# bananaofhappiness/soundscope

Hardware: AMD Instinct MI355X
Metric: audio samples/s analyzed (48 kHz stereo) (higher is better)
Workload: dtype f32 + f64

## Files before the change

soundscope_amd/csrc/ss_fft.hip:

```cpp
#include "ss_kernels.h"
#include "ss_fft_dev.h"
#include <cstdlib>
#include <type_traits>

namespace ssk {

constexpr int kFftPairwWaves = 3;
constexpr int kFftWaves = 2;

constexpr int kX2Stride = 17;
constexpr int kRowB = 17;
constexpr int kPlaneB = 16 * kRowB;
#define X1B(ka, tb_, ta_) ((ka) * kPlaneB + (tb_) * kRowB + (ta_))
#define X2B(kb, ka_, tb_) ((kb) * kPlaneB + (ka_) * kRowB + (tb_))

#define SPEC_POS(k) ((k) ^ (((k) >> 5) & 3))

constexpr uint32_t kColStride = 516;
typedef __attribute__((address_space(3))) float lds_f32;
typedef __attribute__((address_space(3))) char lds_char;
__device__ __forceinline__ void lds_fmax(lds_f32 *p, float v) { (void)__hip_atomic_fetch_max(p, v, __ATOMIC_RELAXED, __HIP_MEMORY_SCOPE_WORKGROUP); }
template <bool LDS_TABLE = false, bool COLS = false>
__device__ __forceinline__ void fft4096_epilogue(const v2f *xb, int t, uint32_t first_bin, uint32_t n_bins,
                                                 float db_offset, const float *__restrict__ offpink,
                                                 float *o_mid, float *o_side, bool store_side = true,
                                                 float side_off = 0.0f, float *colbuf = nullptr, const uint2 *coltab = nullptr,
                                                 const uint2 *colbins = nullptr)
{
    const uint32_t ngroups = (n_bins + 3) >> 2;
    constexpr float kDb = 3.01029995663981195f;
    const float lg0 = __uint_as_float((uint32_t)__builtin_amdgcn_readfirstlane((int)__float_as_uint((-150.0f - db_offset) / kDb)));
    float4 op[2];
#pragma unroll
    for (int i = 0; i < 2; i++) {
        const uint32_t g = (uint32_t)t + 256u * i;
        op[i] = make_float4(0.f, 0.f, 0.f, 0.f);
        uint32_t boff = 16u * g;
        asm volatile("" : "+v"(boff));
        if (!LDS_TABLE && g < ngroups) op[i] = *reinterpret_cast<const float4 *>(reinterpret_cast<const char *>(offpink) + boff);
    }
    float rm[2][4], rs[2][4];
    lds_char *const cb = (lds_char *)colbuf;
    auto fold_group = [&](const int i, const uint32_t g) {
                const uint2 ct = coltab[g];
                const uint32_t o0 = ct.x & 0xFFFFu, o3 = ct.x >> 16, nf = ct.y;
                const bool general = nf == 0u;
                if (__builtin_expect(__ballot(general) != 0ull, 0)) {
                    if (general) {
                        uint32_t gg = g;
                        asm volatile("" : "+v"(gg));
                        const uint2 cw = colbins[gg];
                        const uint32_t o[4] = {cw.x & 0xFFFFu, cw.x >> 16, cw.y & 0xFFFFu, cw.y >> 16};
#pragma unroll
                        for (int e = 0; e < 4; e++) {
                            lds_f32 *a = (lds_f32 *)(cb + o[e]);
                            lds_fmax(a, rm[i][e]);
                            lds_fmax(a + kColStride, rs[i][e]);
                        }
                    }
                }
                if (!general) {
                    const bool p1 = nf > 1u, p2 = nf > 2u, p3 = nf > 3u;
                    auto max3 = [](float a, float b, float c) -> float { float r; asm("v_max3_f32 %0, %1, %2, %3" : "=v"(r) : "v"(a), "v"(b), "v"(c)); return r; };
                    auto max2 = [](float a, float b) -> float { float r; asm("v_max_f32 %0, %1, %2" : "=v"(r) : "v"(a), "v"(b)); return r; };
#pragma unroll
                    for (int row = 0; row < 2; row++) {
                        const float *r = row ? rs[i] : rm[i];
                        float f = max3(r[0], p1 ? r[1] : r[0], p2 ? r[2] : r[0]);
                        f = max2(f, p3 ? r[3] : r[0]);
                        const float l = max3(r[3], p2 ? r[3] : r[2], p1 ? r[3] : r[1]);
                        lds_fmax((lds_f32 *)(cb + o0) + row * kColStride, f);
                        if (!p3) lds_fmax((lds_f32 *)(cb + o3) + row * kColStride, l);
                    }
                }
    };
#pragma unroll
    for (int i = 0; i < 2; i++) {
        const uint32_t g = (uint32_t)t + 256u * i;
        if (g < ngroups) {
            uint32_t k0 = first_bin + 4 * g;
            if (COLS && i == 1) asm volatile("" : "+v"(k0));
            v2f zk[4], zm[4];
#pragma unroll
            for (int e = 0; e < 4; e++) {
                const uint32_t k = k0 + e;
                zk[e] = xb[SPEC_POS(k)];
                zm[e] = xb[SPEC_POS(4096 - k)];
            }
            if (LDS_TABLE) op[i] = reinterpret_cast<const float4 *>(offpink)[g];
#if defined(__HIP_DEVICE_COMPILE__)
            __builtin_amdgcn_sched_barrier(0);
#endif
            float qm[4], qs[4];
#pragma unroll
            for (int e = 0; e < 4; e++) {
                v2f P = zk[e] + zm[e], Q, t, qq;
                asm("v_pk_add_f32 %0, %1, %2 op_sel:[1,1] op_sel_hi:[0,0] neg_lo:[0,1] neg_hi:[0,1]" : "=v"(Q) : "v"(zk[e]), "v"(zm[e]));
                asm("v_pk_mul_f32 %0, %1, %1" : "=v"(t) : "v"(Q));
                asm("v_pk_fma_f32 %0, %1, %1, %2" : "=v"(qq) : "v"(P), "v"(t));
                qm[e] = qq.x;
                qs[e] = qq.y;
            }
            const float opv[4] = {op[i].x, op[i].y, op[i].z, op[i].w};
            const v2f so2 = {side_off, side_off};
            const v2f osa = v2f{op[i].x, op[i].y} + so2, osb = v2f{op[i].z, op[i].w} + so2;
            const float ops[4] = {osa.x, osa.y, osb.x, osb.y};
            const float qmin = fminf(fminf(fminf(qm[0], qm[1]), fminf(qm[2], qm[3])), fminf(fminf(qs[0], qs[1]), fminf(qs[2], qs[3])));
            if (__builtin_expect(__ballot(qmin == 0.0f) == 0ull, 1)) {
#pragma unroll
                for (int e = 0; e < 4; e++) {
                    rm[i][e] = fmaf(__log2f(qm[e]), kDb, opv[e]);
                    rs[i][e] = fmaf(__log2f(qs[e]), kDb, ops[e]);
                }
            } else {
#pragma unroll
                for (int e = 0; e < 4; e++) {
                    rm[i][e] = fmaf(qm[e] == 0.0f ? lg0 : __log2f(qm[e]), kDb, opv[e]);
                    rs[i][e] = qs[e] == 0.0f ? fmaf(lg0, kDb, opv[e]) : fmaf(__log2f(qs[e]), kDb, ops[e]);
                }
            }
            if (COLS) fold_group(i, g);
        } else {
#pragma unroll
            for (int e = 0; e < 4; e++) { rm[i][e] = 0.0f; rs[i][e] = 0.0f; }
        }
    }
    if (COLS) return;
#if defined(__HIP_DEVICE_COMPILE__)
    __builtin_amdgcn_sched_barrier(0);
#endif
#pragma unroll
    for (int i = 0; i < 2; i++) {
        const uint32_t g = (uint32_t)t + 256u * i;
        if (g < ngroups) {
            reinterpret_cast<float4 *>(o_mid)[g] = make_float4(rm[i][0], rm[i][1], rm[i][2], rm[i][3]);
            if (store_side) reinterpret_cast<float4 *>(o_side)[g] = make_float4(rs[i][0], rs[i][1], rs[i][2], rs[i][3]);
        }
    }
}

__device__ __forceinline__ void fft4096_nan_rows(int t, uint32_t n_bins, float *o_first, float *o_second, bool first_nan, bool second_nan)
{
    const uint32_t ngroups = (n_bins + 3) >> 2;
    __builtin_amdgcn_s_waitcnt(0);
    const float qn = __builtin_nanf("");
    for (uint32_t g = (uint32_t)t; g < ngroups; g += 256u) {
        if (first_nan) reinterpret_cast<float4 *>(o_first)[g] = make_float4(qn, qn, qn, qn);
        if (second_nan) reinterpret_cast<float4 *>(o_second)[g] = make_float4(qn, qn, qn, qn);
    }
}

__device__ __forceinline__ void fft4096_floor_rows(int t, uint32_t n_bins, float db_offset, const float *__restrict__ offpink,
                                                float *o_first, float *o_second, bool first_zero, bool second_zero)
{
    const uint32_t ngroups = (n_bins + 3) >> 2;
    __builtin_amdgcn_s_waitcnt(0);
    for (uint32_t g = (uint32_t)t; g < ngroups; g += 256u) {
        const float4 op = *reinterpret_cast<const float4 *>(offpink + 4 * g);
        const float4 v = make_float4(-150.0f + (op.x - db_offset), -150.0f + (op.y - db_offset), -150.0f + (op.z - db_offset), -150.0f + (op.w - db_offset));
        if (first_zero) reinterpret_cast<float4 *>(o_first)[g] = v;
        if (second_zero) reinterpret_cast<float4 *>(o_second)[g] = v;
    }
}

__device__ __forceinline__ void fft4096_floor_columns(int t, uint32_t n_bins, float db_offset, const float *__restrict__ offpink,
                                                      float *colbuf, const uint16_t *bincol, const float *col_init, uint32_t cols,
                                                      bool first_zero, bool second_zero)
{
    __syncthreads();
    for (uint32_t c = (uint32_t)t; c < cols; c += 256u) {
        if (first_zero) colbuf[c] = col_init[c];
        if (second_zero) colbuf[kColStride + c] = col_init[c];
    }
    __syncthreads();
    for (uint32_t k = (uint32_t)t; k < n_bins; k += 256u) {
        const uint32_t c = bincol[k];
        const float v = -150.0f + (offpink[k] - db_offset);
        if (first_zero) lds_fmax((lds_f32 *)colbuf + c, v);
        if (second_zero) lds_fmax((lds_f32 *)colbuf + kColStride + c, v);
    }
}

__device__ __forceinline__ uint32_t umax(uint32_t a, uint32_t b) { return a > b ? a : b; }
__device__ __forceinline__ uint32_t wave_umax_lane63(uint32_t v)
{
#define SS_UMAX_DPP(ctrl, rows) v = umax(v, (uint32_t)__builtin_amdgcn_update_dpp(0, (int)v, ctrl, rows, 0xF, true))
    SS_UMAX_DPP(0x111, 0xF);
    SS_UMAX_DPP(0x112, 0xF);
    SS_UMAX_DPP(0x114, 0xF);
    SS_UMAX_DPP(0x118, 0xF);
    SS_UMAX_DPP(0x142, 0xA);
    SS_UMAX_DPP(0x143, 0xC);
#undef SS_UMAX_DPP
    return v;
}
__device__ __forceinline__ float wave_fsum_lane63(float v)
{
#define SS_FSUM_DPP(ctrl, rows) v += __int_as_float(__builtin_amdgcn_update_dpp(0, __float_as_int(v), ctrl, rows, 0xF, true))
    SS_FSUM_DPP(0x111, 0xF);
    SS_FSUM_DPP(0x112, 0xF);
    SS_FSUM_DPP(0x114, 0xF);
    SS_FSUM_DPP(0x118, 0xF);
    SS_FSUM_DPP(0x142, 0xA);
    SS_FSUM_DPP(0x143, 0xC);
#undef SS_FSUM_DPP
    return v;
}
__device__ __forceinline__ int block_exp_energy(uint32_t a, uint32_t b)
{
    const int e = ((int)a - (int)b + (1 << 23)) >> 24;
    return e < -60 ? -60 : (e > 60 ? 60 : e);
}
__device__ __forceinline__ void read_energies2(const uint32_t (*lv)[2], uint32_t &a, uint32_t &b)
{
    const uint4 q0 = *reinterpret_cast<const uint4 *>(&lv[0][0]), q1 = *reinterpret_cast<const uint4 *>(&lv[2][0]);
    const float sa = (__uint_as_float(q0.x) + __uint_as_float(q0.z)) + (__uint_as_float(q1.x) + __uint_as_float(q1.z));
    const float sb = (__uint_as_float(q0.y) + __uint_as_float(q0.w)) + (__uint_as_float(q1.y) + __uint_as_float(q1.w));
    a = (uint32_t)__builtin_amdgcn_readfirstlane((int)__float_as_uint(sa));
    b = (uint32_t)__builtin_amdgcn_readfirstlane((int)__float_as_uint(sb));
}
__device__ __forceinline__ int block_exp(uint32_t a, uint32_t b)
{
    const int e = ((int)a - (int)b + (1 << 22)) >> 23;
    return e < -60 ? -60 : (e > 60 ? 60 : e);
}
__device__ __forceinline__ float exp2i(int e) { return __uint_as_float((uint32_t)(127 + e) << 23); }
__device__ __forceinline__ float uniform_f(float v) { return __uint_as_float((uint32_t)__builtin_amdgcn_readfirstlane((int)__float_as_uint(v))); }
__device__ __forceinline__ float block_off(int e) { return uniform_f((float)e * -6.02059991327962390f); }
__device__ __forceinline__ void read_levels2(const uint32_t (*lv)[2], uint32_t &a, uint32_t &b)
{
    const uint4 q0 = *reinterpret_cast<const uint4 *>(&lv[0][0]), q1 = *reinterpret_cast<const uint4 *>(&lv[2][0]);
    a = (uint32_t)__builtin_amdgcn_readfirstlane((int)umax(umax(q0.x, q0.z), umax(q1.x, q1.z)));
    b = (uint32_t)__builtin_amdgcn_readfirstlane((int)umax(umax(q0.y, q0.w), umax(q1.y, q1.w)));
}
__device__ __forceinline__ void read_levels4(const uint32_t (*lv)[8], uint32_t (&x)[4])
{
    const uint4 q0 = *reinterpret_cast<const uint4 *>(&lv[0][0]), q1 = *reinterpret_cast<const uint4 *>(&lv[1][0]);
    const uint4 q2 = *reinterpret_cast<const uint4 *>(&lv[2][0]), q3 = *reinterpret_cast<const uint4 *>(&lv[3][0]);
    x[0] = (uint32_t)__builtin_amdgcn_readfirstlane((int)umax(umax(q0.x, q1.x), umax(q2.x, q3.x)));
    x[1] = (uint32_t)__builtin_amdgcn_readfirstlane((int)umax(umax(q0.y, q1.y), umax(q2.y, q3.y)));
    x[2] = (uint32_t)__builtin_amdgcn_readfirstlane((int)umax(umax(q0.z, q1.z), umax(q2.z, q3.z)));
    x[3] = (uint32_t)__builtin_amdgcn_readfirstlane((int)umax(umax(q0.w, q1.w), umax(q2.w, q3.w)));
}
__device__ __forceinline__ void read_energies4(const uint32_t (*lv)[8], uint32_t (&g)[4])
{
    const uint4 e0 = *reinterpret_cast<const uint4 *>(&lv[0][4]), e1 = *reinterpret_cast<const uint4 *>(&lv[1][4]);
    const uint4 e2 = *reinterpret_cast<const uint4 *>(&lv[2][4]), e3 = *reinterpret_cast<const uint4 *>(&lv[3][4]);
    auto fs = [](uint32_t a, uint32_t b, uint32_t c, uint32_t d) -> uint32_t {
        return (uint32_t)__builtin_amdgcn_readfirstlane((int)__float_as_uint((__uint_as_float(a) + __uint_as_float(b)) + (__uint_as_float(c) + __uint_as_float(d))));
    };
    g[0] = fs(e0.x, e1.x, e2.x, e3.x); g[1] = fs(e0.y, e1.y, e2.y, e3.y);
    g[2] = fs(e0.z, e1.z, e2.z, e3.z); g[3] = fs(e0.w, e1.w, e2.w, e3.w);
}
__device__ __forceinline__ int exact_block_exp(uint32_t xa, uint32_t xb, uint32_t ga, uint32_t gb)
{
    if (xa == 0u || xb == 0u) return 0;
    const bool gok = ga != 0u && gb != 0u && ga < 0x7F800000u && gb < 0x7F800000u;
    return gok ? block_exp_energy(ga, gb) : block_exp(xa, xb);
}

// ... 169 lines not shown
struct PhaseMark {
    uint64_t pt = __builtin_amdgcn_s_memtime(), acc[12] = {0, 0, 0, 0, 0, 0, 0, 0, 0, 0, 0, 0};
    __device__ __forceinline__ void operator()(int i) { const uint64_t n = __builtin_amdgcn_s_memtime(); acc[i] += n - pt; pt = n; }
    __device__ __forceinline__ void end() const
    {
        if ((threadIdx.x & 63) != 0) return;
#pragma unroll
        for (int i = 0; i < 12; i++) atomicAdd(&g_fft_prof[i], (unsigned long long)acc[i]);
        atomicAdd(&g_fft_prof[15], 1ull);
    }
};
#else
typedef NoMark PhaseMark;
#endif

template <bool PRIO>
__device__ __forceinline__ void r16_fft(v2f (&z)[16])
{
    if (PRIO) SS_PRIO_LO();
    fft16(z);
    if (PRIO) SS_PRIO_HI();
}
template <class Mark>
__device__ __forceinline__ void r16_row_load(v2f (&z)[16], const v2f *row, Mark &mark, int i)
{
#pragma unroll
    for (int j = 0; j < 16; j++) z[j] = lds_ld64(&row[j]);
    mark(i);
    __syncthreads();
    mark(i + 1);
}
template <bool PRIO, class Mark>
__device__ __forceinline__ void r16_pass2(v2f (&z)[16], const v2f *row, v2f *x2, const v2f *twp, Mark &mark)
{
    r16_row_load(z, row, mark, 2);
    r16_fft<PRIO>(z);
    x2[0] = z[R16(0)];
    v2f twa[4], twb[4];
#pragma unroll
    for (int j = 0; j < 4; j++) twa[j] = lds_ld64(&twp[16 * (1 + j)]);
#pragma unroll
    for (int g = 0; g < 4; g++) {
        const int kb0 = 1 + 4 * g, nk = g == 3 ? 3 : 4;
        if (g < 3) {
#pragma unroll
            for (int j = 0; j < 4; j++) if (kb0 + 4 + j < 16) twb[j] = lds_ld64(&twp[16 * (kb0 + 4 + j)]);
        }
        __builtin_amdgcn_sched_barrier(0);
#pragma unroll
        for (int j = 0; j < nk; j++) x2[(kb0 + j) * kPlaneB] = pk_cmul(z[R16(kb0 + j)], twa[j]);
        __builtin_amdgcn_sched_barrier(0);
#pragma unroll
        for (int j = 0; j < 4; j++) twa[j] = twb[j];
    }
}

constexpr int kMs1Tw = 12;
template <int HS, int TWN, bool COLS>
__global__ __launch_bounds__(256, 3) void k_fft4096_ms1(FftBatchParams p)
{
    constexpr int NH = 16 / HS;
    __shared__ __attribute__((aligned(16))) v2f xbuf[16 * kPlaneB];
    __shared__ __attribute__((aligned(16))) v2f tw2s[256];
    __shared__ __attribute__((aligned(16))) uint32_t hoplev[NH][4][2];
    __shared__ __attribute__((aligned(16))) uint32_t xlev[4][2];
    __shared__ __attribute__((aligned(16))) float offp[2048];
    __shared__ __attribute__((aligned(16))) uint2 coltab[COLS ? 512 : 1];
    __shared__ __attribute__((aligned(16))) float colbuf[COLS ? 2 * kColStride : 1];
    const int t = threadIdx.x;
    WindowRun run;
    if (!window_run(p, run)) return;
    const uint32_t stream = run.stream, w_begin = run.begin, w_end = run.end;
    const float2 *src = reinterpret_cast<const float2 *>(p.pcm) + (size_t)stream * p.frames_per_stream +
                        p.first_start + (size_t)w_begin * p.hop;
    const v2f *twn = reinterpret_cast<const v2f *>(p.tw_n);
    v2f hwp[8];
#pragma unroll
    for (int j = 0; j < 8; j++) hwp[j] = v2f{p.half_window[t + 256 * (2 * j)], p.half_window[t + 256 * (2 * j + 1)]};
    v2f tw1[16];
    r16_load_tw1<TWN>(tw1, twn, t);
    tw2s[t] = reinterpret_cast<const v2f *>(p.tw_256)[(t & 15) * (t >> 4)];
    if (COLS) {
        for (uint32_t g = (uint32_t)t; 4u * g < p.bin_stride; g += 256u) coltab[g] = p.col_groups[g];
        for (uint32_t c = (uint32_t)t; c < p.cols; c += 256u) { const float v = p.col_init[c]; colbuf[c] = v; colbuf[kColStride + c] = v; }
        if (t < 4) { colbuf[512 + t] = 0.0f; colbuf[kColStride + 512 + t] = 0.0f; }
    }
    for (uint32_t g = (uint32_t)t; 4u * g < p.bin_stride; g += 256u)
        reinterpret_cast<float4 *>(offp)[g] = reinterpret_cast<const float4 *>(p.offpink)[g];
    const float cgain = COLS ? (p.integrated ? -13.0f - (float)p.integrated[stream] : p.gain_db) : 0.0f;
    auto flush_columns = [&](uint32_t wdone) {
        float *oc = p.out_cols + ((size_t)stream * p.n_windows + wdone) * 2u * p.cols;
        for (uint32_t c = (uint32_t)t; c < 2u * p.cols; c += 256u) {
            const uint32_t i = c < p.cols ? c : c - p.cols + kColStride;
            const float k = colbuf[i];
            const bool none = k != k;
            if (!none) colbuf[i] = -INFINITY;
            oc[c] = none ? k : fminf(fmaxf(k + cgain, -100.0f), 0.0f);
        }
    };
    const int tb = t & 15, hi = t >> 4;
    const int tsw = SPEC_POS(t);
    const size_t out_win_stride = (size_t)2 * p.bin_stride;
    float *outp = p.out + ((size_t)stream * p.n_windows + w_begin) * out_win_stride;
    v2f sd[16];
#pragma unroll
    for (int j = 0; j < 16; j++) sd[j] = pk_sum_diff(reinterpret_cast<const v2f *>(src)[t + 256 * j]);
    auto windowed = [&](int j) -> v2f { return (j & 1) ? pk_mul_bcast<1>(sd[j], hwp[j >> 1]) : pk_mul_bcast<0>(sd[j], hwp[j >> 1]); };
    const uint32_t wvid = (uint32_t)__builtin_amdgcn_readfirstlane(t >> 6);
    const bool lane63 = (t & 63) == 63;
#pragma unroll
    for (int g = 0; g < NH; g++) {
        float m = 0.0f, d = 0.0f;
#pragma unroll
        for (int q = 0; q < HS; q++) { m = fmaxf(m, fabsf(sd[g * HS + q].x)); d = fmaxf(d, fabsf(sd[g * HS + q].y)); }
        const uint32_t wm = wave_umax_lane63(__float_as_uint(m)), wd = wave_umax_lane63(__float_as_uint(d));
        if (lane63) *reinterpret_cast<uint2 *>(hoplev[(g + 1) % NH][wvid]) = make_uint2(wm, wd);
    }
    __syncthreads();
    uint32_t Pm[NH], Pd[NH];
    Pm[0] = 0u; Pd[0] = 0u;
#pragma unroll
    for (int g = 1; g < NH; g++) read_levels2(hoplev[g], Pm[g], Pd[g]);
    int E = 0;
    float scE = 1.0f, soffE = 0.0f;
    auto rescale = [&](int T) -> float {
        const int dE = T - E;
        if (dE < 2 && dE > -2) return 1.0f;
        const float sc = exp2i(dE);
#pragma unroll
        for (int j = 0; j < 16; j++) sd[j].y *= sc;
        E = T; scE = exp2i(E); soffE = block_off(E);
        return sc;
    };
    bool inner_ok = false;
    uint32_t thr_m = 0u, thr_d = 0u;
    auto presettle = [&]() {
        uint32_t mm = 0u, md = 0u;
#pragma unroll
        for (int g = 2; g < NH; g++) { mm = umax(mm, Pm[g]); md = umax(md, Pd[g]); }
        thr_m = mm + 0x800000u; thr_d = md + 0x800000u;
        inner_ok = mm != 0u && md != 0u && Pm[1] <= thr_m && Pd[1] <= thr_d;
        if (mm != 0u && md != 0u) rescale(block_exp(mm, md));
    };
    presettle();
    PhaseMark mark;
    for (uint32_t w = w_begin; w < w_end; ++w) {
        float2 nx[HS];
        const bool more = (w + 1 < w_end);
        if (COLS && w != w_begin) flush_columns(w - 1);
        const uint4 lq0 = *reinterpret_cast<const uint4 *>(&hoplev[0][0][0]), lq1 = *reinterpret_cast<const uint4 *>(&hoplev[0][2][0]);
        __builtin_amdgcn_sched_barrier(0);
        v2f z[16];
#pragma unroll
        for (int j = 0; j < 16; j++) z[j] = windowed(j);
        __builtin_amdgcn_sched_barrier(0);
        const uint32_t nPm = (uint32_t)__builtin_amdgcn_readfirstlane((int)umax(umax(lq0.x, lq0.z), umax(lq1.x, lq1.z)));
        const uint32_t nPd = (uint32_t)__builtin_amdgcn_readfirstlane((int)umax(umax(lq0.y, lq0.w), umax(lq1.y, lq1.w)));
#pragma unroll
        for (int g = 0; g < NH - 1; g++) { Pm[g] = Pm[g + 1]; Pd[g] = Pd[g + 1]; }
        Pm[NH - 1] = nPm; Pd[NH - 1] = nPd;
        bool zrow_m = false, zrow_d = false;
        if (__builtin_expect(!inner_ok || nPm > thr_m || nPd > thr_d, 0)) {
            uint32_t am = 0u, ad = 0u;
#pragma unroll
            for (int g = 0; g < NH; g++) { am |= Pm[g]; ad |= Pd[g]; }
            zrow_m = am == 0u; zrow_d = ad == 0u;
            if (!(zrow_m || zrow_d)) {
                float xm = 0.0f, xd = 0.0f;
#pragma unroll
                for (int j = 0; j < 16; j++) { xm = fmaf(z[j].x, z[j].x, xm); xd = fmaf(z[j].y, z[j].y, xd); }
                const float wm = wave_fsum_lane63(xm), wd = wave_fsum_lane63(xd);
                if (lane63) *reinterpret_cast<uint2 *>(xlev[wvid]) = make_uint2(__float_as_uint(wm), __float_as_uint(wd));
                __syncthreads();
                uint32_t Xm, Xd;
                read_energies2(xlev, Xm, Xd);
                if (Xm != 0u && Xd != 0u && Xm < 0x7F800000u && Xd < 0x7F800000u) {
                    int T = E + block_exp_energy(Xm, Xd);
                    T = T < -60 ? -60 : (T > 60 ? 60 : T);
                    const float sc = rescale(T);
#pragma unroll
                    for (int j = 0; j < 16; j++) z[j].y *= sc;
                }
            }
        }
        const float soff = soffE;
        r16_fft<true>(z);
        xbuf[X1B(0, tb, hi)] = z[R16(0)];
#pragma unroll
        for (int ka = 1; ka < 16; ka++) xbuf[X1B(ka, tb, hi)] = r16_pass1_tw<TWN>(ka, z[R16(ka)], tw1);
#pragma unroll
        for (int q = 0; q < HS; q++) {
            nx[q] = make_float2(0.f, 0.f);
            if (more) nx[q] = src[(size_t)(w + 1 - w_begin) * p.hop + t + 256 * (16 - HS + q)];
        }
        mark(0);
        __syncthreads();
        mark(1);
        r16_pass2<true>(z, &xbuf[X1B(hi, tb, 0)], &xbuf[X2B(0, hi, tb)], tw2s + tb, mark);
        mark(4);
        __syncthreads();
        mark(5);
        r16_row_load(z, &xbuf[X1B(hi, tb, 0)], mark, 6);
        r16_fft<true>(z);
#pragma unroll
        for (int kc = 0; kc < 16; kc++)
            if ((p.publish_mask >> kc) & 1u) xbuf[kc * 256 + tsw] = z[R16(kc)];
        mark(8);
        __syncthreads();
        mark(9);
        SS_PRIO_LO();
        if (more) {
#pragma unroll
            for (int j = 0; j < 16 - HS; j++) sd[j] = sd[j + HS];
            float m = 0.0f, d = 0.0f;
#pragma unroll
            for (int q = 0; q < HS; q++) {
                const v2f v = pk_sum_diff(v2f{nx[q].x, nx[q].y});
                m = fmaxf(m, fabsf(v.x)); d = fmaxf(d, fabsf(v.y));
                sd[16 - HS + q] = v2f{v.x, v.y * scE};
            }
            const uint32_t wm = wave_umax_lane63(__float_as_uint(m)), wd = wave_umax_lane63(__float_as_uint(d));
            if (lane63) *reinterpret_cast<uint2 *>(hoplev[0][wvid]) = make_uint2(wm, wd);
            presettle();
        }
        float *o_mid = outp + (size_t)(w - w_begin) * out_win_stride;
        fft4096_epilogue<true, COLS>(xbuf, t, p.first_bin, p.n_bins, p.db_offset, offp, o_mid, o_mid + p.bin_stride, true, soff, colbuf, coltab, p.col_bins);
        if (__builtin_expect(zrow_m || zrow_d, 0) && xbuf[SPEC_POS(p.first_bin)].x == xbuf[SPEC_POS(p.first_bin)].x) {
            if (!COLS) fft4096_floor_rows(t, p.n_bins, p.db_offset, p.offpink, o_mid, o_mid + p.bin_stride, zrow_m, zrow_d);
            else fft4096_floor_columns(t, p.n_bins, p.db_offset, p.offpink, colbuf, p.bin_col, p.col_init, p.cols, zrow_m, zrow_d);
        }
        mark(10);
        __syncthreads();
        mark(11);
    }
    mark.end();
    if (COLS) flush_columns(w_end - 1);
}

__global__ __launch_bounds__(256, kFftPairwWaves) void k_fft4096_pairw(FftBatchParams p, uint32_t fft_ch)
{
    __shared__ __attribute__((aligned(16))) v2f xbuf[16 * kPlaneB];
    __shared__ __attribute__((aligned(16))) v2f tw2s[256];
    __shared__ __attribute__((aligned(16))) uint32_t hoplev[5][4];
    __shared__ __attribute__((aligned(16))) uint32_t xlev[4][2];
    const int t = threadIdx.x;
    const uint32_t pairs_per_block = p.windows_per_block >> 1;
    const uint32_t n_pairs_max = (p.n_windows + 1) >> 1;
    const uint32_t groups = (n_pairs_max + pairs_per_block - 1) / pairs_per_block;
    uint32_t bid = xcd_logical_id();
    if (bid >= p.n_streams * groups * fft_ch) return;
    const uint32_t ch = bid % fft_ch; bid /= fft_ch;
    const uint32_t grp = bid % groups;
    const uint32_t stream = bid / groups;
    const uint32_t n_win = p.windows_of ? p.windows_of[stream] : p.n_windows;
    const uint32_t n_pairs = (n_win + 1) >> 1;
    const uint32_t pp_begin = grp * pairs_per_block;
    uint32_t pp_end = pp_begin + pairs_per_block;
    if (pp_begin >= n_pairs) return;
    if (pp_end > n_pairs) pp_end = n_pairs;
    const uint32_t C = p.channels;
    const float *src = p.pcm + ((size_t)stream * p.frames_per_stream + p.first_start + (size_t)pp_begin * 2048u) * C + ch;
    const v2f *twn = reinterpret_cast<const v2f *>(p.tw_n);
    float hw[16], hw2[16];
#pragma unroll
    for (int j = 0; j < 16; j++) hw2[j] = hw[j] = p.window[t + 256 * j];
    v2f tw1[16];
    r16_load_tw1<6>(tw1, twn, t);
    tw1[5] = twn[5 * t]; tw1[6] = twn[6 * t]; tw1[7] = twn[7 * t];
    tw2s[t] = reinterpret_cast<const v2f *>(p.tw_256)[(t & 15) * (t >> 4)];
    const int tb = t & 15, hi = t >> 4;
    const int tsw = SPEC_POS(t);
    const size_t row_stride = (size_t)fft_ch * p.bin_stride;
    float *outp = p.out + (((size_t)stream * p.n_windows + 2u * pp_begin) * fft_ch + ch) * p.bin_stride;
    float raw[20];
    const bool two0 = (2u * pp_begin + 1u < n_win);
#pragma unroll
    for (int j = 0; j < 20; j++) raw[j] = (j < 16 || two0) ? src[(size_t)(t + 256 * j) * C] : 0.0f;
    const uint32_t wvid = (uint32_t)__builtin_amdgcn_readfirstlane(t >> 6);
    const bool lane63 = (t & 63) == 63;
    auto hop_level = [&](float a, float b, float c, float d) -> uint32_t {
        const uint32_t ua = __float_as_uint(a) & 0x7FFFFFFFu, ub = __float_as_uint(b) & 0x7FFFFFFFu;
        const uint32_t uc = __float_as_uint(c) & 0x7FFFFFFFu, ud = __float_as_uint(d) & 0x7FFFFFFFu;
        return wave_umax_lane63(umax(umax(ua, ub), umax(uc, ud)));
    };
    auto read_level = [&](const uint32_t *lv) -> uint32_t {
        const uint4 q = *reinterpret_cast<const uint4 *>(lv);
        return (uint32_t)__builtin_amdgcn_readfirstlane((int)umax(umax(q.x, q.y), umax(q.z, q.w)));
    };
#pragma unroll
    for (int g = 0; g < 5; g++) {
        const uint32_t wl = hop_level(raw[4 * g], raw[4 * g + 1], raw[4 * g + 2], raw[4 * g + 3]);
        if (lane63) hoplev[g][wvid] = wl;
    }
    __syncthreads();
    uint32_t P[5];
#pragma unroll
    for (int g = 0; g < 5; g++) P[g] = read_level(hoplev[g]);
    int E = 0;
    auto settle = [&]() {
        if ((P[0] | P[1] | P[2] | P[3]) == 0u || (P[1] | P[2] | P[3] | P[4]) == 0u) return;
        if (umax(umax(umax(P[0], P[1]), umax(P[2], P[3])), P[4]) >= 0x7F800000u) return;
        const uint32_t ma = umax(P[1], P[2]), ea = umax(P[0], P[3]), mb = umax(P[2], P[3]), eb = umax(P[1], P[4]);
        int T;
        if (ma != 0u && mb != 0u && ea <= ma + 0x800000u && eb <= mb + 0x800000u) {
            T = block_exp(ma, mb);
        } else {
            float xa = 0.0f, xb = 0.0f;
#pragma unroll
            for (int j = 0; j < 16; j++) { const float pa = raw[j] * hw[j], pb = raw[j + 4] * hw[j]; xa = fmaf(pa, pa, xa); xb = fmaf(pb, pb, xb); }
            const float wa = wave_fsum_lane63(xa), wb = wave_fsum_lane63(xb);
            if (lane63) *reinterpret_cast<uint2 *>(xlev[wvid]) = make_uint2(__float_as_uint(wa), __float_as_uint(wb));
            __syncthreads();
            uint32_t Xa, Xb;
            read_energies2(xlev, Xa, Xb);
            if (Xa == 0u || Xb == 0u || Xa >= 0x7F800000u || Xb >= 0x7F800000u) return;
            T = block_exp_energy(Xa, Xb);
        }
        const int dE = T - E;
        if (dE >= 2 || dE <= -2) {
            const float sc = exp2i(T);
#pragma unroll
            for (int j = 0; j < 16; j++) hw2[j] = hw[j] * sc;
            E = T;
        }
    };
    settle();
    NoMark nomark;
    for (uint32_t pp = pp_begin; pp < pp_end; ++pp) {
        const bool two = (2u * pp + 1u < n_win);
        const bool more = (pp + 1 < pp_end);
        const bool more2 = more && (2u * pp + 3u < n_win);
        const bool zrow_a = (P[0] | P[1] | P[2] | P[3]) == 0u, zrow_b = (P[1] | P[2] | P[3] | P[4]) == 0u;
        float nx[8];
        const float *nsrc = src + ((size_t)(pp - pp_begin) * 2048u + t) * C;
#pragma unroll
        for (int q = 0; q < 8; q++) {
            nx[q] = 0.0f;
            if (q < 4 ? more : more2) nx[q] = nsrc[(size_t)(256 * (20 + q)) * C];
        }
// ... 678 lines not shown
```

soundscope_amd/csrc/ss_fft_dev.h:

```cpp
#pragma once
#include "ss_kernels.h"

namespace ssk {

__device__ __forceinline__ float2 cadd(float2 a, float2 b) { return make_float2(a.x + b.x, a.y + b.y); }
__device__ __forceinline__ float2 csub(float2 a, float2 b) { return make_float2(a.x - b.x, a.y - b.y); }
__device__ __forceinline__ float2 cmul(float2 a, float2 w) { return make_float2(a.x * w.x - a.y * w.y, a.x * w.y + a.y * w.x); }
__device__ __forceinline__ float2 cmul_cs(float2 a, float c, float s) { return make_float2(a.x * c + a.y * s, a.y * c - a.x * s); }
__device__ __forceinline__ float2 cmul_mi(float2 a) { return make_float2(a.y, -a.x); }

typedef float v2f __attribute__((ext_vector_type(2)));
__device__ __forceinline__ v2f lds_ld64(const v2f *p)
{
    return *(const volatile __attribute__((address_space(3))) v2f *)p;
}
__device__ __forceinline__ v2f pk_sub_ib(v2f a, v2f b)
{
    v2f r;
    asm("v_pk_add_f32 %0, %1, %2 op_sel:[0,1] op_sel_hi:[1,0] neg_lo:[0,0] neg_hi:[0,1]" : "=v"(r) : "v"(a), "v"(b));
    return r;
}
__device__ __forceinline__ v2f pk_add_ib(v2f a, v2f b)
{
    v2f r;
    asm("v_pk_add_f32 %0, %1, %2 op_sel:[0,1] op_sel_hi:[1,0] neg_lo:[0,1] neg_hi:[0,0]" : "=v"(r) : "v"(a), "v"(b));
    return r;
}
__device__ __forceinline__ v2f pk_cmul(v2f a, v2f w)
{
    v2f m, r;
    asm("v_pk_mul_f32 %1, %2, %3 op_sel:[1,1] op_sel_hi:[1,0]\n\t"
        "v_pk_fma_f32 %0, %2, %3, %1 op_sel:[0,0,0] op_sel_hi:[0,1,1] neg_lo:[0,0,1] neg_hi:[0,0,0]"
        : "=v"(r), "=&v"(m) : "v"(a), "v"(w));
    return r;
}
__device__ __forceinline__ v2f pk_cmul_k(v2f a, v2f w)
{
    v2f m, r;
    asm("v_pk_mul_f32 %1, %2, %3 op_sel:[1,1] op_sel_hi:[1,0]\n\t"
        "v_pk_fma_f32 %0, %2, %3, %1 op_sel:[0,0,0] op_sel_hi:[0,1,1] neg_lo:[0,0,1] neg_hi:[0,0,0]"
        : "=v"(r), "=&v"(m) : "v"(a), "s"(w));
    return r;
}
__device__ __forceinline__ v2f pk_w2pre(v2f a) { return pk_sub_ib(a, a); }
__device__ __forceinline__ v2f pk_w6pre(v2f a)
{
    v2f r;
    asm("v_pk_add_f32 %0, %1, %1 op_sel:[1,0] op_sel_hi:[0,1] neg_lo:[0,1] neg_hi:[1,1]" : "=v"(r) : "v"(a));
    return r;
}
__device__ __forceinline__ v2f pk_mul_mi(v2f a)
{
    v2f r;
    const v2f zero = {0.0f, 0.0f};
    asm("v_pk_add_f32 %0, %1, %2 op_sel:[0,1] op_sel_hi:[1,0] neg_lo:[0,0] neg_hi:[0,1]" : "=v"(r) : "v"(zero), "v"(a));
    return r;
}

template <int S>
__device__ __forceinline__ v2f pk_mul_bcast(v2f a, v2f w)
{
    v2f r;
    if (S == 0) asm("v_pk_mul_f32 %0, %1, %2 op_sel:[0,0] op_sel_hi:[1,0]" : "=v"(r) : "v"(a), "v"(w));
    else asm("v_pk_mul_f32 %0, %1, %2 op_sel:[0,1] op_sel_hi:[1,1]" : "=v"(r) : "v"(a), "v"(w));
    return r;
}
__device__ __forceinline__ v2f pk_sum_diff(v2f f)
{
    v2f r;
    asm("v_pk_add_f32 %0, %1, %1 op_sel:[0,1] op_sel_hi:[0,1] neg_lo:[0,0] neg_hi:[0,1]" : "=v"(r) : "v"(f));
    return r;
}

__device__ __forceinline__ void radix4(v2f &a0, v2f &a1, v2f &a2, v2f &a3)
{
    const v2f t0 = a0 + a2, t1 = a0 - a2, t2 = a1 + a3, t3 = a1 - a3;
    a0 = t0 + t2;
    a2 = t0 - t2;
    a1 = pk_sub_ib(t1, t3);
    a3 = pk_add_ib(t1, t3);
}

#define R16(k) ((((k) & 3) << 2) | ((k) >> 2))
__device__ __forceinline__ void fft16(v2f (&a)[16])
{
    constexpr float C1 = 0.92387953251128674f, S1 = 0.38268343236508977f, R = 0.70710678118654752f;
    const v2f w1 = {C1, -S1}, w3 = {S1, -C1}, w9 = {-C1, S1};
    radix4(a[0], a[4], a[8], a[12]);
    radix4(a[1], a[5], a[9], a[13]);
    radix4(a[2], a[6], a[10], a[14]);
    radix4(a[3], a[7], a[11], a[15]);
    a[5] = pk_cmul_k(a[5], w1);
    a[9] = pk_w2pre(a[9]) * R;
    a[13] = pk_cmul_k(a[13], w3);
    a[6] = pk_w2pre(a[6]) * R;
    a[10] = pk_mul_mi(a[10]);
    a[14] = pk_w6pre(a[14]) * R;
    a[7] = pk_cmul_k(a[7], w3);
    a[11] = pk_w6pre(a[11]) * R;
    a[15] = pk_cmul_k(a[15], w9);
    radix4(a[0], a[1], a[2], a[3]);
    radix4(a[4], a[5], a[6], a[7]);
    radix4(a[8], a[9], a[10], a[11]);
    radix4(a[12], a[13], a[14], a[15]);
}

template <int TWN>
constexpr bool r16_resident(int ka)
{
    static_assert(TWN == 6 || TWN == 9 || TWN == 12, "resident pass-1 twiddles: 6, 9 or 12");
    return (ka & 3) == 0 || (ka & 12) == 0 || (TWN >= 9 && (ka >> 2) == 1) || (TWN >= 12 && (ka >> 2) == 2);
}
template <int TWN>
__device__ __forceinline__ void r16_load_tw1(v2f (&tw)[16], const v2f *w4096, int t)
{
#pragma unroll
    for (int ka = 1; ka < 16; ka++) if (r16_resident<TWN>(ka)) tw[ka] = w4096[ka * t];
}
template <int TWN>
__device__ __forceinline__ v2f r16_pass1_tw(int ka, v2f v, const v2f (&tw)[16])
{
    if (TWN > 6 && r16_resident<TWN>(ka)) return pk_cmul(v, tw[ka]);
    if (ka & 3) v = pk_cmul(v, tw[ka & 3]);
    if (ka & 12) v = pk_cmul(v, tw[ka & 12]);
    return v;
}

__device__ __forceinline__ float db_from_sq(float q, float off)
{
    float r = fmaf(__log2f(q), 3.01029995663981195f, off);
    return q == 0.0f ? -150.0f : r;
}


constexpr int kX1Stride = 272;
constexpr int kRow = 18;
constexpr int kPlane = 16 * kRow;

constexpr int kFft16kLdsBytes = (2 * 16 * kPlane + 256) * 8;
template <class Src>
__device__ __forceinline__ void fft16k_transform(const FftBatchParams &p, Src &src, void *lds)
{
    v2f (*const xbuf2)[16 * kPlane] = reinterpret_cast<v2f (*)[16 * kPlane]>(lds);
    v2f *const tw2s = reinterpret_cast<v2f *>(lds) + 2 * 16 * kPlane;
#define X1W(ka, tb_, ta_) ((ka) * kX1Stride + (tb_) + 16 * (ta_))
#define X2W(kb, ka_, tb_) ((kb) * kPlane + (ka_) * kRow + (tb_))
    const int q = threadIdx.x >> 8;
    const int t = threadIdx.x & 255;
    v2f *xbuf = xbuf2[q];
    if (!src.begin()) return;
    const v2f *tw16k = reinterpret_cast<const v2f *>(p.tw_n);
    const v2f *tw4k = reinterpret_cast<const v2f *>(p.tw_core);
    if (threadIdx.x < 256) tw2s[t] = reinterpret_cast<const v2f *>(p.tw_256)[t];

    v2f z[16];
#pragma unroll
    for (int j = 0; j < 16; j++) {
        const uint32_t i = (uint32_t)t + 256u * j;
        const v2f a = src.load(i), b = src.load(i + 4096u);
        z[j] = q ? pk_cmul(a - b, tw16k[2 * i]) : a + b;
    }
    const int tb = t & 15, hi = t >> 4;
    v2f twg[16];
    r16_load_tw1<6>(twg, tw4k, t);
    fft16(z);
    xbuf[X1W(0, tb, hi)] = z[R16(0)];
#pragma unroll
    for (int ka = 1; ka < 16; ka++) xbuf[X1W(ka, tb, hi)] = r16_pass1_tw<6>(ka, z[R16(ka)], twg);
    src.loaded();
    __syncthreads();
#pragma unroll
    for (int ta = 0; ta < 16; ta++) z[ta] = xbuf[X1W(hi, tb, ta)];
    __syncthreads();
    fft16(z);
    xbuf[X2W(0, hi, tb)] = z[R16(0)];
#pragma unroll
    for (int kb = 1; kb < 16; kb++) xbuf[X2W(kb, hi, tb)] = pk_cmul(z[R16(kb)], tw2s[tb * kb]);
    __syncthreads();
#pragma unroll
    for (int qq = 0; qq < 16; qq++) z[qq] = xbuf[X2W(hi, tb, qq)];
    __syncthreads();
    fft16(z);
#pragma unroll
    for (int kc = 0; kc < 16; kc++) xbuf[kc * 256 + t] = z[R16(kc)];
    __syncthreads();
    const auto store = src.row();
    constexpr int kAhead = 8;
    for (uint32_t idx0 = threadIdx.x; idx0 < p.n_bins; idx0 += 512u * kAhead) {
        v2f wv[kAhead];
        float pk[kAhead];
#pragma unroll
        for (int m = 0; m < kAhead; m++) {
            const uint32_t idx = idx0 + 512u * (uint32_t)m;
            const uint32_t ic = idx < p.n_bins ? idx : p.n_bins - 1u;
            const uint32_t b = p.first_bin + ic;
            wv[m] = tw16k[b < 8192u ? b : 0u];
            pk[m] = p.pink ? p.pink[ic] : 0.0f;
        }
#pragma unroll
        for (int m = 0; m < kAhead; m++) {
            const uint32_t idx = idx0 + 512u * (uint32_t)m;
            if (idx >= p.n_bins) break;
            const uint32_t b = p.first_bin + idx;
            float xr, xi;
            if (b == 8192u) {
                const v2f z0 = xbuf2[0][0];
                xr = z0.x - z0.y; xi = 0.0f;
            } else {
                const uint32_t qb = b & 1u, k = b >> 1;
                const uint32_t km = qb ? (4095u - k) : ((4096u - k) & 4095u);
                const v2f zk = xbuf2[qb][k];
                const v2f zc = xbuf2[qb][km];
                const float sr = (zk.x + zc.x) * 0.5f, si = (zk.y - zc.y) * 0.5f;
                const float dr = (zk.x - zc.x) * 0.5f, di = (zk.y + zc.y) * 0.5f;
                const float tr = wv[m].x * dr - wv[m].y * di;
                const float ti = wv[m].x * di + wv[m].y * dr;
                xr = sr + ti;
                xi = si - tr;
            }
            const float qv = fmaf(xr, xr, xi * xi);
            float r = fmaf(__log2f(qv), 3.01029995663981195f, p.db_offset);
            r = (qv == 0.0f) ? -150.0f : r;
            store(idx, r, pk[m]);
        }
    }
    src.done();
#undef X1W
#undef X2W
}

struct Fft16kFlat {
    const FftBatchParams &p;
    int midside;
    uint32_t fft_ch, bid;
    uint32_t ch, w, stream;
    const float *base;
    __device__ __forceinline__ bool begin()
    {
        ch = bid % fft_ch; bid /= fft_ch;
        w = bid % p.n_windows;
        stream = bid / p.n_windows;
        if (p.windows_of && w >= p.windows_of[stream]) return false;
        const size_t start = p.first_start + (size_t)w * p.hop;
        base = p.pcm + ((size_t)stream * p.frames_per_stream + start) * p.channels;
        return true;
    }
    __device__ __forceinline__ v2f load(uint32_t i) const
    {
        float x0, x1;
        if (midside) {
            const float2 va = reinterpret_cast<const float2 *>(base)[2 * (size_t)i];
            const float2 vb = reinterpret_cast<const float2 *>(base)[2 * (size_t)i + 1];
            x0 = ch == 0 ? (va.x + va.y) * 0.5f : (va.x - va.y) * 0.5f;
            x1 = ch == 0 ? (vb.x + vb.y) * 0.5f : (vb.x - vb.y) * 0.5f;
        } else if (p.channels == 1) {
            const float2 v = reinterpret_cast<const float2 *>(base)[i];
            x0 = v.x; x1 = v.y;
// ... 31 lines not shown
```

Measured before the change: 209.1 billion.

## Fuse window multiply into first radix-4 stage and hand-schedule FFT16 second stage

Only the first eight windowed inputs are loaded up front. The windowing of the upper eight is folded into the first radix-4 butterflies through packed FMAs on raw samples (sd/hwp), and windowed(j) is recomputed on the rare energy-rescale path. The second FFT16 stage is rewritten as inline-asm blocks that fold the twiddles into FMAs with tangent-factored constants, and the zero-check min chain is rewritten as min3. The aim is to cut VALU instructions and register pressure in the per-hop FFT, at the risk of subtle numerical or ordering differences and a fragile asm schedule; the rescale path now scales only z[0..7], which relies on sd/hwp having been rescaled elsewhere.

```diff
diff --git a/soundscope_amd/csrc/ss_fft.hip b/soundscope_amd/csrc/ss_fft.hip
--- a/soundscope_amd/csrc/ss_fft.hip
+++ b/soundscope_amd/csrc/ss_fft.hip
@@ -105,7 +105,8 @@
             const v2f so2 = {side_off, side_off};
             const v2f osa = v2f{op[i].x, op[i].y} + so2, osb = v2f{op[i].z, op[i].w} + so2;
             const float ops[4] = {osa.x, osa.y, osb.x, osb.y};
-            const float qmin = fminf(fminf(fminf(qm[0], qm[1]), fminf(qm[2], qm[3])), fminf(fminf(qs[0], qs[1]), fminf(qs[2], qs[3])));
+            auto min3 = [](float a, float b, float c) -> float { return __builtin_fminf(__builtin_fminf(a, b), c); };
+            const float qmin = fminf(min3(min3(min3(qm[0], qm[1], qm[2]), qm[3], qs[0]), qs[1], qs[2]), qs[3]);
             if (__builtin_expect(__ballot(qmin == 0.0f) == 0ull, 1)) {
 #pragma unroll
                 for (int e = 0; e < 4; e++) {
@@ -581,7 +582,7 @@
         __builtin_amdgcn_sched_barrier(0);
         v2f z[16];
 #pragma unroll
-        for (int j = 0; j < 16; j++) z[j] = windowed(j);
+        for (int j = 0; j < 8; j++) z[j] = windowed(j);
         __builtin_amdgcn_sched_barrier(0);
         const uint32_t nPm = (uint32_t)__builtin_amdgcn_readfirstlane((int)umax(umax(lq0.x, lq0.z), umax(lq1.x, lq1.z)));
         const uint32_t nPd = (uint32_t)__builtin_amdgcn_readfirstlane((int)umax(umax(lq0.y, lq0.w), umax(lq1.y, lq1.w)));
@@ -597,7 +598,7 @@
             if (!(zrow_m || zrow_d)) {
                 float xm = 0.0f, xd = 0.0f;
 #pragma unroll
-                for (int j = 0; j < 16; j++) { xm = fmaf(z[j].x, z[j].x, xm); xd = fmaf(z[j].y, z[j].y, xd); }
+                for (int j = 0; j < 16; j++) { const v2f v = j < 8 ? z[j] : windowed(j); xm = fmaf(v.x, v.x, xm); xd = fmaf(v.y, v.y, xd); }
                 const float wm = wave_fsum_lane63(xm), wd = wave_fsum_lane63(xd);
                 if (lane63) *reinterpret_cast<uint2 *>(xlev[wvid]) = make_uint2(__float_as_uint(wm), __float_as_uint(wd));
                 __syncthreads();
@@ -608,12 +609,19 @@
                     T = T < -60 ? -60 : (T > 60 ? 60 : T);
                     const float sc = rescale(T);
 #pragma unroll
-                    for (int j = 0; j < 16; j++) z[j].y *= sc;
+                    for (int j = 0; j < 8; j++) z[j].y *= sc;
                 }
             }
         }
         const float soff = soffE;
-        r16_fft<true>(z);
+        SS_PRIO_LO();
+#pragma unroll
+        for (int r = 0; r < 4; r++) {
+            if (r & 1) radix4_windowed<1>(z[r], z[r + 4], z[r + 8], z[r + 12], sd[r + 8], hwp[(r + 8) >> 1], sd[r + 12], hwp[(r + 12) >> 1]);
+            else radix4_windowed<0>(z[r], z[r + 4], z[r + 8], z[r + 12], sd[r + 8], hwp[(r + 8) >> 1], sd[r + 12], hwp[(r + 12) >> 1]);
+        }
+        fft16_stage2(z);
+        SS_PRIO_HI();
         xbuf[X1B(0, tb, hi)] = z[R16(0)];
 #pragma unroll
         for (int ka = 1; ka < 16; ka++) xbuf[X1B(ka, tb, hi)] = r16_pass1_tw<TWN>(ka, z[R16(ka)], tw1);
diff --git a/soundscope_amd/csrc/ss_fft_dev.h b/soundscope_amd/csrc/ss_fft_dev.h
--- a/soundscope_amd/csrc/ss_fft_dev.h
+++ b/soundscope_amd/csrc/ss_fft_dev.h
@@ -34,14 +34,6 @@
         : "=v"(r), "=&v"(m) : "v"(a), "v"(w));
     return r;
 }
-__device__ __forceinline__ v2f pk_cmul_k(v2f a, v2f w)
-{
-    v2f m, r;
-    asm("v_pk_mul_f32 %1, %2, %3 op_sel:[1,1] op_sel_hi:[1,0]\n\t"
-        "v_pk_fma_f32 %0, %2, %3, %1 op_sel:[0,0,0] op_sel_hi:[0,1,1] neg_lo:[0,0,1] neg_hi:[0,0,0]"
-        : "=v"(r), "=&v"(m) : "v"(a), "s"(w));
-    return r;
-}
 __device__ __forceinline__ v2f pk_w2pre(v2f a) { return pk_sub_ib(a, a); }
 __device__ __forceinline__ v2f pk_w6pre(v2f a)
 {
@@ -49,14 +41,6 @@
     asm("v_pk_add_f32 %0, %1, %1 op_sel:[1,0] op_sel_hi:[0,1] neg_lo:[0,1] neg_hi:[1,1]" : "=v"(r) : "v"(a));
     return r;
 }
-__device__ __forceinline__ v2f pk_mul_mi(v2f a)
-{
-    v2f r;
-    const v2f zero = {0.0f, 0.0f};
-    asm("v_pk_add_f32 %0, %1, %2 op_sel:[0,1] op_sel_hi:[1,0] neg_lo:[0,0] neg_hi:[0,1]" : "=v"(r) : "v"(zero), "v"(a));
-    return r;
-}
-
 template <int S>
 __device__ __forceinline__ v2f pk_mul_bcast(v2f a, v2f w)
 {
@@ -81,28 +65,86 @@
     a3 = pk_add_ib(t1, t3);
 }
 
+#define SS_PK_SUB_IB(D, A, B) "v_pk_add_f32 " D ", " A ", " B " op_sel:[0,1] op_sel_hi:[1,0] neg_lo:[0,0] neg_hi:[0,1]\n\t"
+#define SS_PK_ADD_IB(D, A, B) "v_pk_add_f32 " D ", " A ", " B " op_sel:[0,1] op_sel_hi:[1,0] neg_lo:[0,1] neg_hi:[0,0]\n\t"
+#define SS_PK_W6PRE(D, A) "v_pk_add_f32 " D ", " A ", " A " op_sel:[1,0] op_sel_hi:[0,1] neg_lo:[0,1] neg_hi:[1,1]\n\t"
+#define SS_PK_ADD(D, A, B) "v_pk_add_f32 " D ", " A ", " B "\n\t"
+#define SS_PK_SUB(D, A, B) "v_pk_add_f32 " D ", " A ", " B " neg_lo:[0,1] neg_hi:[0,1]\n\t"
+#define SS_PK_FMA(D, V, K, T) "v_pk_fma_f32 " D ", " V ", " K ", " T "\n\t"
+#define SS_PK_FNMA(D, V, K, T) "v_pk_fma_f32 " D ", " V ", " K ", " T " neg_lo:[1,0,0] neg_hi:[1,0,0]\n\t"
+#define SS_PK_FMA_SUB_IK(D, V, K, T) "v_pk_fma_f32 " D ", " V ", " K ", " T " op_sel:[1,0,0] op_sel_hi:[0,1,1] neg_lo:[0,0,0] neg_hi:[1,0,0]\n\t"
+#define SS_PK_FMA_ADD_IK(D, V, K, T) "v_pk_fma_f32 " D ", " V ", " K ", " T " op_sel:[1,0,0] op_sel_hi:[0,1,1] neg_lo:[1,0,0] neg_hi:[0,0,0]\n\t"
 #define R16(k) ((((k) & 3) << 2) | ((k) >> 2))
+__device__ __forceinline__ void fft16_stage2(v2f (&a)[16])
+{
+    constexpr float C1 = 0.92387953251128674f, T1 = 0.41421356237309505f, R = 0.70710678118654752f;
+    const v2f kc = {C1, C1}, kt = {T1, T1}, kr = {R, R};
+    v2f tmp;
+    radix4(a[0], a[1], a[2], a[3]);
+    asm(SS_PK_FMA_SUB_IK("%1", "%1", "%5", "%1")
+        SS_PK_FMA_ADD_IK("%3", "%3", "%5", "%3")
+        SS_PK_SUB_IB("%2", "%2", "%2")
+        SS_PK_ADD_IB("%4", "%1", "%3")
+        SS_PK_SUB_IB("%3", "%1", "%3")
+        SS_PK_FNMA("%1", "%2", "%7", "%0")
+        SS_PK_FMA("%2", "%2", "%7", "%0")
+        SS_PK_FMA("%0", "%3", "%6", "%2")
+        SS_PK_FNMA("%2", "%3", "%6", "%2")
+        SS_PK_FMA_ADD_IK("%3", "%4", "%6", "%1")
+        SS_PK_FMA_SUB_IK("%1", "%4", "%6", "%1")
+        : "+v"(a[4]), "+v"(a[5]), "+v"(a[6]), "+v"(a[7]), "=&v"(tmp) : "s"(kt), "s"(kc), "s"(kr));
+    asm(SS_PK_SUB_IB("%1", "%1", "%1")
+        SS_PK_W6PRE("%3", "%3")
+        SS_PK_SUB_IB("%4", "%0", "%2")
+        SS_PK_ADD_IB("%2", "%0", "%2")
+        SS_PK_ADD("%0", "%1", "%3")
+        SS_PK_SUB("%1", "%1", "%3")
+        SS_PK_FNMA("%3", "%0", "%5", "%4")
+        SS_PK_FMA("%0", "%0", "%5", "%4")
+        SS_PK_FMA_ADD_IK("%4", "%1", "%5", "%2")
+        SS_PK_FMA_SUB_IK("%1", "%1", "%5", "%2")
+        : "+v"(a[8]), "+v"(a[9]), "+v"(a[10]), "+v"(a[11]), "=&v"(tmp) : "s"(kr));
+    a[10] = a[11];
+    a[11] = tmp;
+    asm(SS_PK_FMA_ADD_IK("%1", "%1", "%5", "%1")
+        SS_PK_FMA_SUB_IK("%3", "%3", "%5", "%3")
+        SS_PK_W6PRE("%2", "%2")
+        SS_PK_SUB_IB("%4", "%3", "%1")
+        SS_PK_ADD_IB("%3", "%3", "%1")
+        SS_PK_FNMA("%1", "%2", "%7", "%0")
+        SS_PK_FMA("%2", "%2", "%7", "%0")
+        SS_PK_FNMA("%0", "%3", "%6", "%2")
+        SS_PK_FMA("%2", "%3", "%6", "%2")
+        SS_PK_FMA_ADD_IK("%3", "%4", "%6", "%1")
+        SS_PK_FMA_SUB_IK("%1", "%4", "%6", "%1")
+        : "+v"(a[12]), "+v"(a[13]), "+v"(a[14]), "+v"(a[15]), "=&v"(tmp) : "s"(kt), "s"(kc), "s"(kr));
+}
+
 __device__ __forceinline__ void fft16(v2f (&a)[16])
 {
-    constexpr float C1 = 0.92387953251128674f, S1 = 0.38268343236508977f, R = 0.70710678118654752f;
-    const v2f w1 = {C1, -S1}, w3 = {S1, -C1}, w9 = {-C1, S1};
     radix4(a[0], a[4], a[8], a[12]);
     radix4(a[1], a[5], a[9], a[13]);
     radix4(a[2], a[6], a[10], a[14]);
     radix4(a[3], a[7], a[11], a[15]);
-    a[5] = pk_cmul_k(a[5], w1);
-    a[9] = pk_w2pre(a[9]) * R;
-    a[13] = pk_cmul_k(a[13], w3);
-    a[6] = pk_w2pre(a[6]) * R;
-    a[10] = pk_mul_mi(a[10]);
-    a[14] = pk_w6pre(a[14]) * R;
-    a[7] = pk_cmul_k(a[7], w3);
-    a[11] = pk_w6pre(a[11]) * R;
-    a[15] = pk_cmul_k(a[15], w9);
-    radix4(a[0], a[1], a[2], a[3]);
-    radix4(a[4], a[5], a[6], a[7]);
-    radix4(a[8], a[9], a[10], a[11]);
-    radix4(a[12], a[13], a[14], a[15]);
+    fft16_stage2(a);
+}
+template <int S>
+__device__ __forceinline__ void radix4_windowed(v2f &a0, v2f &a1, v2f &a2, v2f &a3, v2f sc, v2f hc, v2f sd, v2f hd)
+{
+#define SS_WIN_FMA(D, V, H, T, NEG) "v_pk_fma_f32 " D ", " V ", " H ", " T " op_sel:[0,%c9,0] op_sel_hi:[1,%c9,1]" NEG "\n\t"
+    v2f o0, m1 = a1;
+    asm(SS_WIN_FMA("%2", "%5", "%6", "%0", "")
+        SS_WIN_FMA("%0", "%5", "%6", "%0", " neg_lo:[1,0,0] neg_hi:[1,0,0]")
+        SS_WIN_FMA("%3", "%7", "%8", "%1", "")
+        SS_WIN_FMA("%1", "%7", "%8", "%1", " neg_lo:[1,0,0] neg_hi:[1,0,0]")
+        SS_PK_ADD("%4", "%2", "%3")
+        SS_PK_SUB("%2", "%2", "%3")
+        SS_PK_ADD_IB("%3", "%0", "%1")
+        SS_PK_SUB_IB("%0", "%0", "%1")
+        : "+v"(a0), "+v"(m1), "=&v"(a2), "=&v"(a3), "=&v"(o0) : "v"(sc), "v"(hc), "v"(sd), "v"(hd), "n"(S));
+    a1 = a0;
+    a0 = o0;
+#undef SS_WIN_FMA
 }
 
 template <int TWN>
```

Result: faster. 213.0 billion (median of 6 runs) (+1.9%).
